# speedcell4/torchrua

Hardware: AMD Instinct MI355X
Metric: pack->reduce throughput, 65536 seqs/GPU h=512 bf16 (M elements/s) + % HBM roofline (higher is better)
Workload: dtype bf16; 1 GPU; pack->reduce_sum: 65536 seqs/GPU, len~U(8,512), hidden=512, bf16 (north-star shape; N=17046960 rows on rank 0); ranks_reported_by_process_group=1, cpus_of_rank0=256, torch_threads_rank0=16, numa_node_of_rank0_gpu=0

## Files before the change

### include/rua.h

```cpp
#ifndef RUA_H_
#define RUA_H_

#include <stdint.h>

#ifdef __cplusplus
extern "C" {
#endif

#define RUA_ABI_VERSION 6

#define RUA_EINVAL   (-1)
#define RUA_EALIGN   (-2)
#define RUA_ERANGE   (-3)

enum rua_kind { RUA_CAT = 0, RUA_LEFT = 1, RUA_PACK = 2, RUA_RIGHT = 3, RUA_LIST = 4 };

typedef struct rua_layout {
  int32_t kind;
  int32_t tile_t_log2;
  int64_t n_rows;
  int64_t B;
  int64_t T_phys;
  int64_t T_log;
  const int64_t* lens;
// ... 50 lines not shown
int rua_move_rows(const rua_layout* dst, const rua_layout* src, int32_t tmap, int64_t tmap_arg,
                  void* dst_data, const void* src_data, int64_t row_bytes,
                  const void* fill16, int64_t pad_row, int32_t flags, void* stream);

int rua_setitem_backward(const rua_layout* list, const rua_layout* src, const void* grad, void* grad_value,
                         void* grad_raw, int64_t row_bytes, int32_t flags, void* stream);

enum rua_dtype {
  RUA_F32 = 0, RUA_BF16 = 1, RUA_F16 = 2, RUA_F64 = 3,
  RUA_I64 = 4, RUA_I32 = 5, RUA_I16 = 6, RUA_I8 = 7, RUA_U8 = 8
};
#define RUA_TIES_FINAL 2
#define RUA_BWD_FILL_PADDING 0x100
#define RUA_BWD_TIES_POSITIVE 0x200
enum rua_op {
  RUA_SUM = 0, RUA_MEAN = 1, RUA_MAX = 2, RUA_MIN = 3, RUA_PROD = 4, RUA_LOGSUMEXP = 5
};

#define RUA_EXTREME_WORDS    1027
#define RUA_OP_SCRATCH_CLEAN 0x100
#define RUA_OP_NO_EMPTY      0x200
#define RUA_OP_SHORT_SEQS    0x400
int64_t rua_reduce_ws_bytes(int64_t n_rows, int64_t H, int32_t dtype, int64_t split_rows);
int rua_reduce_team_waves(int64_t n_rows, int64_t B, int64_t row_bytes);
int rua_segment_reduce(const rua_layout* lay, const int64_t* perm, const void* data, void* out,
                       int64_t H, int32_t dtype, int32_t op, int32_t include_self,
                       uint64_t empty_bits, void* extreme, int64_t split_rows, void* ws, void* ties_out,
                       void* stream);

int rua_pack_reduce(const rua_layout* src, const rua_layout* pack, const void* data, void* pack_data, void* out,
                    int64_t H, int32_t dtype, int32_t op, uint64_t empty_bits, void* extreme, int64_t split_rows,
                    void* ws, void* stream);

int rua_pack_sums(const rua_layout* src, const rua_layout* pack, const void* data, void* pack_data, float* sums,
                  int64_t H, int32_t dtype, int64_t split_rows, void* ws, void* stream);

int rua_pack_sums_backward(const rua_layout* src, const rua_layout* pack, const void* grad_pack, const float* grad_sums,
                           void* grad_src, int64_t H, int32_t dtype, void* stream);

int rua_sums_cast(const void* in, void* out, int64_t n, int32_t dtype, int32_t to_f32, void* stream);

int rua_segment_reduce_backward(const rua_layout* lay, const int64_t* perm, const void* data, const void* out,
                                const void* grad_out, void* grad_in, int64_t H, int32_t dtype, int32_t op,
                                int32_t include_self, int64_t split_rows, void* ws, void* ties,
                                const void* self_in, void* stream);

int rua_scatter_self_grad(const int64_t* counts, int64_t S, int64_t H, const void* self_in, const void* out,
                          const void* grad_out, const void* aux, void* grad_self, int32_t dtype, int32_t op,
                          int32_t include_self, void* stream);

int64_t rua_softmax_ws_bytes(const rua_layout* lay, int64_t H, int32_t dtype);
int rua_segment_softmax(const rua_layout* lay, const void* data, void* out, int64_t H, int32_t dtype, int32_t log,
                        void* ws, void* stream);
int rua_segment_softmax_backward(const rua_layout* lay, const void* y, const void* grad_out, void* grad_in, int64_t H,
                                 int32_t dtype, int32_t log, void* ws, void* stream);

#define RUA_POOL_OUT_ACC 0x100
int64_t rua_softmax_pool_ws_bytes(const rua_layout* lay, int64_t H, int64_t D, int32_t dtype);
int rua_segment_softmax_pool(const rua_layout* lay, const void* values, const void* scores, void* out, void* lse,
                             int64_t H, int64_t D, int32_t dtype, void* ws, void* stream);
int rua_segment_softmax_pool_backward(const rua_layout* lay, const void* grad_out, const void* values,
                                      const void* scores, const void* out, const void* lse, void* grad_values,
                                      void* grad_scores, int64_t H, int64_t D, int32_t dtype, void* ws, void* stream);

#define RUA_NORM_MEAN_ACC 0x100
int64_t rua_norm_ws_bytes(const rua_layout* lay, int64_t H, int32_t dtype);
// ... 156 lines not shown
```

### torchrua_amd/_lib.py

```python
import ctypes
import os
import threading
from ctypes import POINTER, Structure, c_char_p, c_double, c_int, c_int32, c_int64, c_uint64, c_void_p

import torch

_HERE = os.path.dirname(os.path.abspath(__file__))
LIB_PATH = os.environ.get('RUA_LIB_PATH') or os.path.join(_HERE, 'librua_hip.so')

ABI_VERSION = 6
CAT, LEFT, PACK, RIGHT, LIST = 0, 1, 2, 3, 4
T_SHIFT, T_ROLL, T_REV_S, T_REV_D, T_ZERO = 0, 1, 2, 3, 4
TIES_FINAL = 2
BWD_FILL_PADDING = 0x100
BWD_TIES_POSITIVE = 0x200
MOVE_SCATTER = 1
MOVE_NT_ON, MOVE_NT_OFF = 2, 4
MOVE_XCD_SPAN_ON, MOVE_XCD_SPAN_OFF = 256, 512
MOVE_NO_NARROW = 2048
OP_SCRATCH_CLEAN, OP_NO_EMPTY = 0x100, 0x200
EXTREME_WORDS = 1027
POOL_OUT_ACC = 0x100
NORM_MEAN_ACC = 0x100
OP_SHORT_SEQS = 0x400
CONV_MAX_TAPS = 8
JOIN_MAX_PARTS = 8
RUNS_BITS = 0x100
WINDOW_MAX_K = 64
CRF_MAX_TAGS = 64
CRF_LOG, CRF_MAX = 0, 1
WINDOW_TAKE = 6
F32, BF16, F16, F64 = 0, 1, 2, 3
SUM, MEAN, MAX, MIN, PROD, LOGSUMEXP = 0, 1, 2, 3, 4, 5

I64, I32, I16, I8, U8 = 4, 5, 6, 7, 8

DTYPES = {torch.float32: F32, torch.bfloat16: BF16, torch.float16: F16, torch.float64: F64}
INT_DTYPES = {torch.int64: I64, torch.int32: I32, torch.int16: I16, torch.int8: I8, torch.uint8: U8}
SCAN_DTYPES = {**DTYPES, torch.int64: I64}


class RuaLayout(Structure):
    _fields_ = [
        ('kind', c_int32), ('tile_t_log2', c_int32),
        ('n_rows', c_int64), ('B', c_int64), ('T_phys', c_int64), ('T_log', c_int64),
        ('lens', c_void_p), ('len_add', c_int64), ('off', c_void_p),
        ('boff', c_void_p), ('T', c_int64), ('sorted', c_void_p), ('unsorted', c_void_p),
        ('bptr', c_void_p), ('tptr', c_void_p),
        ('bsz', c_void_p), ('tile_start', c_void_p), ('n_tchunks', c_int64), ('n_tiles', c_int64),
    ]


# ... 200 lines not shown
```

### torchrua_amd/_ops.py

```python
import ctypes
import threading
from typing import Callable, Optional, Sequence, Tuple

import torch
from torch import Tensor
from torch.autograd.function import once_differentiable

from torchrua_amd import _lib as L
from torchrua_amd import _meta as M

_kernel_hook: Optional[Callable[[str, bool], None]] = None


def set_kernel_hook(fn) -> None:
    global _kernel_hook
    _kernel_hook = fn


def _prod(shape) -> int:
    n = 1
    for d in shape:
        n *= d
    return n

# ... 267 lines not shown
        split, ws = split_workspace(lay, H, data.dtype, dev, team_ok=False)
        L.check(lib.rua_segment_reduce_backward(lay.ref(), None, L.ptr(data), L.ptr(out), L.ptr(grad), L.ptr(g), H,
                                                L.DTYPES[data.dtype], op,
                                                (L.TIES_FINAL if ties is not None else 0) | L.BWD_FILL_PADDING | L.BWD_TIES_POSITIVE,
                                                split, L.ptr(ws), L.ptr(ties), None, L.stream_ptr(dev)),
                'rua_segment_reduce_backward')
        ctx.lay, ctx.op, ctx.hidden = lay, op, tuple(out.shape[1:])
        return g

    @staticmethod
    def backward(ctx, gg: Tensor):
        if ctx.op not in (L.SUM, L.MEAN):
            raise RuntimeError('torchrua_amd: prod (and the fused max / min / logsumexp kernel outside create_graph) '
                               'differentiate once; second-order gradients exist for sum, mean, max, min and logsumexp '
                               '(and for every cast, select and gather)')
        return reduce(gg.contiguous(), ctx.lay, ctx.op, ctx.hidden, None), None, None, None, None, None


def reduce(data: Tensor, lay: M.Lay, op: int, hidden, lens: Optional[Tensor]) -> Tensor:
    if data.requires_grad and torch.is_grad_enabled():
        return _Reduce.apply(data.contiguous(), lay, op, tuple(hidden), lens)
    return launch_reduce(lay, _plain(data), op, hidden=tuple(hidden))


SUMS_DTYPES = (torch.float32, torch.bfloat16, torch.float16)
_SUMS_KEY = 'pack_sums'


def pack_sums_can(data: Tensor, hidden: Tuple[int, ...]) -> bool:
    return (data.dtype in SUMS_DTYPES and data.is_contiguous() and data.data_ptr() % 16 == 0 and data.numel() > 0
            and (_prod(hidden) * data.element_size()) % 16 == 0)


def launch_pack_sums(data: Tensor, src: M.Lay, dst: M.Lay, hidden: Tuple[int, ...]) -> Tuple[Tensor, Tensor]:
    dev = data.device
    H = _prod(hidden)
    pdata = torch.empty((dst.n_rows,) + tuple(hidden), dtype=data.dtype, device=dev)
    sums = torch.empty((src.B,) + tuple(hidden), dtype=torch.float32, device=dev)
    split, ws = split_workspace(src, H, data.dtype, dev, team_ok=False)
    _call('to_pack', 'rua_pack_sums', dev, src.ref(), dst.ref(), L.ptr(data), L.ptr(pdata), L.ptr(sums), H,
          L.DTYPES[data.dtype], split, L.ptr(ws))
    return pdata, sums


def launch_sums_cast(x: Tensor, dtype: torch.dtype, to_f32: bool, name: Optional[str] = None) -> Tensor:
    dev = L.require_device(x)
    x = x.contiguous()
    out = torch.empty(x.shape, dtype=torch.float32 if to_f32 else dtype, device=dev)
    args = (L.ptr(x), L.ptr(out), x.numel(), L.DTYPES[dtype], 1 if to_f32 else 0)
    if name is None:
        L.check(L.load().rua_sums_cast(*args, L.stream_ptr(dev)), 'rua_sums_cast')
    else:
        _call(name, 'rua_sums_cast', dev, *args)
    return out


class _SumsCast(torch.autograd.Function):

    @staticmethod
    def forward(ctx, sums: Tensor, dtype: torch.dtype):
        ctx.dtype = dtype
        return launch_sums_cast(sums, dtype, False, name='reduce')

    @staticmethod
    def backward(ctx, grad: Tensor):
        if torch.is_grad_enabled():
            return grad.to(torch.float32), None
        return launch_sums_cast(grad, ctx.dtype, True), None


class _PackSums(torch.autograd.Function):

    @staticmethod
    def forward(ctx, data: Tensor, src: M.Lay, dst: M.Lay, hidden: Tuple[int, ...]):
# ... 1735 lines not shown
```

### torchrua_amd/csrc/rua_pack_sums_plan.h

```cpp
#pragma once
#include <stdint.h>
#include "rua.h"
#include "rua_wave.h"

namespace rua {

inline int pack_sums_check(const rua_layout* src, const rua_layout* pack, int64_t H, int32_t dtype) {
  if (!src || !pack || H < 0 || src->B < 0) return RUA_EINVAL;
  if (dtype != RUA_F32 && dtype != RUA_BF16 && dtype != RUA_F16) return RUA_EINVAL;
  if (src->kind != RUA_CAT && src->kind != RUA_LEFT && src->kind != RUA_RIGHT) return RUA_EINVAL;
  if (src->kind == RUA_CAT && src->lens && !src->off) return RUA_EINVAL;
  if (pack->kind != RUA_PACK || pack->B != src->B || (pack->T > 0 && !pack->boff)) return RUA_EINVAL;
  return 0;
}

struct PackSumsBackwardPlan {
  int err, epl, lp_log2;
  int64_t n_chunks;
  unsigned grid;
};
inline PackSumsBackwardPlan plan_pack_sums_backward(int64_t B, int64_t H, int esize, uintptr_t ptrs) {
  PackSumsBackwardPlan P = {};
  P.epl = 16 / esize;
  if (H % P.epl != 0 || ptrs % 16 != 0) { P.err = RUA_EALIGN; return P; }
  const int64_t lpr = H / P.epl;
  P.lp_log2 = lanes_log2(lpr);
  P.n_chunks = (lpr + RUA_WAVE - 1) / RUA_WAVE;
  if (B > 0x7fffffffLL / (P.n_chunks > 0 ? P.n_chunks : 1)) { P.err = RUA_ERANGE; return P; }
  P.grid = (unsigned)(B * P.n_chunks);
  return P;
}

}
```

### torchrua_amd/csrc/rua_reduce.hip

```cpp
#include <hip/hip_runtime.h>
#include <stdarg.h>
#include <stdio.h>
#include <string.h>
#include <atomic>
#include <deque>
#include <mutex>
#include <string>
#include "rua_reduce_impl.h"
#include "rua_pack_sums_plan.h"

namespace rua {
std::atomic<int> g_trace_on{0};
static std::mutex g_trace_mu;
static std::deque<std::string> g_trace_log;
constexpr size_t TRACE_CAP = 512;
static inline bool tracing() { return g_trace_on.load(std::memory_order_relaxed) != 0; }
void trace_add(const char* rec) {
  std::lock_guard<std::mutex> lk(g_trace_mu);
  if (g_trace_log.size() >= TRACE_CAP) g_trace_log.pop_front();
  g_trace_log.emplace_back(rec);
}
__attribute__((format(printf, 1, 2))) static std::string fmt(const char* f, ...) {
  char buf[320];
  va_list ap;
  va_start(ap, f);
  vsnprintf(buf, sizeof buf, f, ap);
  va_end(ap);
  return buf;
}
static const char* op_name(int op, bool ties) {
  switch (op) {
    case RUA_SUM: return "sum";
    case RUA_MEAN: return "mean";
    case RUA_MAX: return ties ? "max_t" : "max";
    case RUA_MIN: return ties ? "min_t" : "min";
    case RUA_PROD: return "prod";
    case RUA_LOGSUMEXP: return "logsumexp";
  }
  return "?";
}
template <typename Emit>
static void trace_reduce(const ReducePlan& P, const char* tname, Emit&& emit) {
  static const char* const kern[] = {"seg_reduce_ranks_kernel", "seg_reduce_team_kernel", "seg_reduce_kernel"};
  auto rec = [&](const char* k, bool nt, int wpb) {
    emit(fmt("%s T=%s EPL=%d OP=%s NT=%d COPY=%d CPW=%d WPB=%d team=%d glog=%d check=%d split=%d no_empty=%d", k, tname,
             P.epl, op_name(P.op, P.ties), nt ? 1 : 0, P.copy ? 1 : 0, P.cpw, wpb, P.team, P.glog, P.check,
             P.split ? 1 : 0, P.no_empty).c_str());
  };
  rec(kern[P.form], P.nt, P.wpb);
  if (P.split) {
    rec("seg_reduce_tail_kernel", P.nt, 1);
    rec("seg_reduce_combine_kernel", false, COMBINE_WAVES_MAX / P.cpw);
  }
}
template <typename Emit>
static void trace_backward(const BackwardPlan& P, const char* tname, Emit&& emit) {
  static const char* const kern[] = {"seg_backward_rows_kernel", "seg_backward_ranks_kernel", "seg_backward_walk_kernel",
                                     "seg_backward_kernel"};
  for (int k = 0; k < P.n_phases; ++k)
    for (const char* name : {kern[P.form], "seg_backward_tail_kernel"}) {
      emit(fmt("%s T=%s EPL=%d OP=%s NT=%d TV=%d chunks=%d span=%d split=%d phased=%d ties_final=%d pad_memset=%d", name,
               tname, P.epl, op_name(P.op, false), P.nt ? 1 : 0, P.tv[k], P.n_chunks > 1 ? 1 : 0, P.span ? 1 : 0,
               P.do_split ? 1 : 0, P.phased ? 1 : 0, P.ties_final ? 1 : 0, P.pad_memset ? 1 : 0).c_str());
      if (!P.do_split) break;
    }
}

static const ReduceEntry* entry_for(int dtype) {
  switch (dtype) {
    case RUA_F32: return &reduce_entry_f32();
    case RUA_BF16: return &reduce_entry_bf16();
    case RUA_F16: return &reduce_entry_f16();
    case RUA_F64: return &reduce_entry_f64();
  }
  return nullptr;
}

static int dispatch_reduce(int dtype, int op, hipStream_t s, const rua_layout& L, const int64_t* perm, const void* data,
                           void* out, int64_t H, int include_self, uint64_t empty_bits, void* extreme, int64_t split,
                           void* ws, const rua_layout* CD, void* copy, void* ties, int hints, std::string* dry,
                           void* acc_out = nullptr) {
  const ReduceEntry* E = entry_for(dtype);
  if (!E) return RUA_EINVAL;
  const ReducePlan P = plan_reduce(L, E->esize, H, op, include_self, perm != nullptr, ws != nullptr, ties != nullptr,
                                   copy != nullptr,
                                   (uintptr_t)data | (uintptr_t)out | (uintptr_t)copy | (uintptr_t)ties | (uintptr_t)acc_out,
                                   split, hints);
  if (P.err) return P.err;
  if (dry) trace_reduce(P, E->name, [&](const char* r) { dry->append(r).push_back('\n'); });
  else if (tracing()) trace_reduce(P, E->name, trace_add);
  return dry ? 0 : E->reduce(P, s, L, perm, data, out, H, include_self, empty_bits, extreme, ws, CD, copy, ties, acc_out);
}

constexpr int EXTREME_WORDS_ENTRY = RUA_EXTREME_WORDS;
__global__ void extreme_init_entry_kernel(unsigned long long* ext, int want_max_of_data) {
  (void)want_max_of_data;
  for (int i = threadIdx.x; i < EXTREME_WORDS_ENTRY; i += blockDim.x) ext[i] = 0ull;
}
int reduce_int(int dtype, int op, hipStream_t s, const rua_layout& L, const int64_t* perm, const void* data, void* out,
               int64_t H, int include_self, int64_t split, void* ws);
int64_t reduce_int_ws_bytes(int64_t n_rows, int64_t H, int64_t split);

static bool layout_ok(const rua_layout* lay, const int64_t* perm, int64_t H) {
  if (!lay || H < 0 || lay->B < 0) return false;
  if (lay->kind != RUA_CAT && lay->kind != RUA_PACK && lay->kind != RUA_LEFT && lay->kind != RUA_RIGHT) return false;
  if (lay->kind == RUA_CAT && lay->lens && !lay->off) return false;
  if (lay->kind == RUA_PACK && lay->T > 0 && !lay->boff) return false;
  return !perm || lay->kind == RUA_CAT;
}
static int segment_reduce_backward(const rua_layout* lay, const int64_t* perm, const void* data, const void* out,
                                   const void* grad_out, void* grad_in, int64_t H, int32_t dtype, int32_t op,
                                   int32_t include_self, int64_t split_rows, void* ws, void* ties, const void* self_in,
                                   void* stream, std::string* dry) {
  if (!layout_ok(lay, perm, H)) return RUA_EINVAL;
  if (self_in && !perm) return RUA_EINVAL;
  if (lay->B == 0 || H == 0 || lay->n_rows == 0) return 0;
  if (!data || !out || !grad_out || !grad_in) return RUA_EINVAL;
  const bool fill = (include_self & RUA_BWD_FILL_PADDING) != 0;
  const int tie_rule = (include_self & RUA_BWD_TIES_POSITIVE) ? BWD_TIES_POSITIVE : 0;
  include_self &= 0xff;
// ... 126 lines not shown
  if (include_self && op == RUA_PROD && !aux) return RUA_EINVAL;
  hipStream_t s = (hipStream_t)stream;
  const int inc = include_self ? 1 : 0;
  const ReduceEntry* E = entry_for(dtype);
  return E ? E->self_grad(s, counts, S, H, self_in, out, grad_out, aux, grad_self, op, inc) : RUA_EINVAL;
}

int64_t rua_reduce_ws_bytes(int64_t n_rows, int64_t H, int32_t dtype, int64_t split_rows) {
  if (split_rows <= 0 || n_rows <= 0 || H <= 0) return 0;
  if (dtype >= RUA_I64 && dtype <= RUA_U8) return reduce_int_ws_bytes(n_rows, H, split_rows);
  const int64_t acc = dtype == RUA_F64 ? 8 : 4;
  const int64_t max_extra = n_rows / split_rows;
  const int64_t chunks_scalar = (H + RUA_WAVE - 1) / RUA_WAVE;
  const int64_t max_u = max_extra * chunks_scalar;
  const int64_t cols = chunks_scalar * RUA_WAVE * (dtype == RUA_F64 ? 2 : 8);
  return 32 + max_u * 64 + 2 * max_extra * 2 * cols * acc + 256;
}

int rua_segment_reduce(const rua_layout* lay, const int64_t* perm, const void* data, void* out, int64_t H,
                       int32_t dtype, int32_t op, int32_t include_self, uint64_t empty_bits, void* extreme,
                       int64_t split_rows, void* ws, void* ties, void* stream) {
  return segment_reduce(lay, perm, data, out, H, dtype, op, include_self, empty_bits, extreme, split_rows, ws, ties, stream,
                        nullptr);
}

int rua_pack_reduce(const rua_layout* src, const rua_layout* pack, const void* data, void* pack_data, void* out,
                    int64_t H, int32_t dtype, int32_t op, uint64_t empty_bits, void* extreme, int64_t split_rows,
                    void* ws, void* stream) {
  return pack_reduce(src, pack, data, pack_data, out, H, dtype, op, empty_bits, extreme, split_rows, ws, stream, nullptr);
}

int rua_pack_sums(const rua_layout* src, const rua_layout* pack, const void* data, void* pack_data, float* sums,
                  int64_t H, int32_t dtype, int64_t split_rows, void* ws, void* stream) {
  const int rc = pack_sums_check(src, pack, H, dtype);
  if (rc) return rc;
  if (src->B == 0 || H == 0) return 0;
  if (!sums || !pack_data || !data) return RUA_EINVAL;
  return dispatch_reduce(dtype, RUA_SUM, (hipStream_t)stream, *src, nullptr, data, nullptr, H, 0, 0, nullptr, split_rows, ws,
                         pack, pack_data, nullptr, 0, nullptr, sums);
}

int rua_pack_sums_backward(const rua_layout* src, const rua_layout* pack, const void* grad_pack, const float* grad_sums,
                           void* grad_src, int64_t H, int32_t dtype, void* stream) {
  const int rc = pack_sums_check(src, pack, H, dtype);
  if (rc) return rc;
  if (src->B == 0 || H == 0 || src->n_rows == 0) return 0;
  if (!grad_pack || !grad_sums || !grad_src) return RUA_EINVAL;
  const ReduceEntry* E = entry_for(dtype);
  const PackSumsBackwardPlan P = plan_pack_sums_backward(src->B, H, E->esize,
                                                         (uintptr_t)grad_pack | (uintptr_t)grad_sums | (uintptr_t)grad_src);
  if (P.err) return P.err;
  const bool nt = reduce_nt(src->n_rows, H, E->esize);
  if (tracing())
    trace_add(fmt("pack_sums_backward_kernel T=%s EPL=%d NT=%d chunks=%lld", E->name, P.epl, nt ? 1 : 0,
                  (long long)P.n_chunks).c_str());
  return E->pack_sums_backward((hipStream_t)stream, *src, *pack, grad_pack, grad_sums, grad_src, H, P.lp_log2, P.n_chunks, nt);
}

int rua_sums_cast(const void* in, void* out, int64_t n, int32_t dtype, int32_t to_f32, void* stream) {
  if (n < 0 || (dtype != RUA_F32 && dtype != RUA_BF16 && dtype != RUA_F16)) return RUA_EINVAL;
  if (n == 0) return 0;
  if (!in || !out || in == out) return RUA_EINVAL;
  const ReduceEntry* E = entry_for(dtype);
  const uintptr_t narrow = (uintptr_t)(to_f32 ? in : out), wide = (uintptr_t)(to_f32 ? out : in);
  if (narrow % E->esize != 0 || wide % 4 != 0) return RUA_EALIGN;
  return E->sums_cast((hipStream_t)stream, in, out, n, to_f32 ? 1 : 0);
}

int rua_fill_empty(const rua_layout* lay, void* out, int64_t H, int32_t dtype, int32_t op, void* extreme,
                   void* stream) {
  if (!lay || H < 0 || !extreme) return RUA_EINVAL;
  const int reset = (op & RUA_OP_SCRATCH_CLEAN) ? 1 : 0;
// ... 19 lines not shown
```

### torchrua_amd/csrc/rua_reduce_impl.h

```cpp
#pragma once
#include <type_traits>
#include <hip/hip_bf16.h>
#include <hip/hip_fp16.h>
#include "rua_dev.h"
#include "rua_reduce_plan.h"

namespace rua {

constexpr int UNROLL_T = RUA_UNROLL_T;
constexpr int EXTREME_SLOTS = 1024;

template <typename T> struct elem;
template <> struct elem<float> {
  using acc = float;
  static __device__ __forceinline__ float up(float v) { return v; }
  static __device__ __forceinline__ float down(float v) { return v; }
};
template <> struct elem<double> {
  using acc = double;
  static __device__ __forceinline__ double up(double v) { return v; }
  static __device__ __forceinline__ double down(double v) { return v; }
};
template <> struct elem<__hip_bfloat16> {
  using acc = float;
// ... 95 lines not shown

constexpr int RUA_MAX_T = 6, RUA_MIN_T = 7;
constexpr bool op_is_max(int op) { return op == RUA_MAX || op == RUA_MAX_T; }
constexpr bool op_is_min(int op) { return op == RUA_MIN || op == RUA_MIN_T; }
constexpr bool op_counts(int op) { return op == RUA_MAX_T || op == RUA_MIN_T; }
constexpr bool op_uses_aux(int op) { return op == RUA_LOGSUMEXP || op_counts(op); }

template <typename A, bool IS_MAX>
__device__ __forceinline__ void tie_update(A& acc, A& cnt, A x, A c) {
  const bool xn = x != x, an = acc != acc;
  const bool better = xn ? !an : (!an && (IS_MAX ? x > acc : x < acc));
  const bool equal = xn ? an : (x == acc);
  cnt = better ? c : (equal ? cnt + c : cnt);
  acc = better ? x : acc;
}

template <typename A, int EPL>
struct Fold {
  A acc[EPL], aux[EPL];
  A opp;
};

template <typename A, int EPL, int OP>
__device__ __forceinline__ void fold_init(Fold<A, EPL>& f) {
#pragma unroll
  for (int e = 0; e < EPL; ++e) {
    f.acc[e] = (OP == RUA_PROD) ? (A)1 : (op_is_max(OP) || OP == RUA_LOGSUMEXP) ? -acc_inf<A>()
             : op_is_min(OP) ? acc_inf<A>() : (A)0;
    f.aux[e] = (A)0;
  }
  f.opp = op_is_min(OP) ? -acc_inf<A>() : acc_inf<A>();
}

template <typename T, int EPL, int OP, bool NT, bool COPY, int CPW = 1, bool RANKS = false>
__device__ __forceinline__ void fold_rows(const Unit<T, EPL>& U, int64_t t_lo, int64_t t_hi,
                                          const T* __restrict__ data, int64_t H,
                                          Fold<typename elem<T>::acc, EPL * CPW>& f, const rua_layout& CD,
                                          T* __restrict__ copy, int lane, int team_w = 0, int team_n = 1,
                                          bool track = true) {
  using A = typename elem<T>::acc;
  constexpr int UT = CPW == 1 ? UNROLL_T : UNROLL_T / 2;
  constexpr int CW = RUA_WAVE * EPL;
  struct alignas(sizeof(T) * EPL > 8 ? 8 : sizeof(T) * EPL) Pack { T v[EPL]; };
  typedef unsigned int RawV0 __attribute__((ext_vector_type(sizeof(T) * EPL >= 4 ? sizeof(T) * EPL / 4 : 1)));
  typedef RawV0 RawV __attribute__((aligned(sizeof(T) * EPL > 8 ? 8 : (sizeof(T) * EPL >= 4 ? sizeof(T) * EPL : 4))));
  const int rpw = U.rpw, rsub = U.rsub;
  const bool colok = U.colok;
  const int64_t col = U.col, base = U.base, tb = U.tb, L_rows = U.n_rows;
  const int64_t* __restrict__ tbl = U.tbl;

  int64_t tv = (tbl && t_lo + lane < t_hi) ? tbl[tb + t_lo + lane] : 0;
  int64_t cv = (COPY && t_lo + lane < t_hi) ? CD.boff[t_lo + lane] : 0;
  for (int64_t tblk = t_lo; tblk < t_hi; tblk += RUA_WAVE) {
    const int64_t nxt = tblk + RUA_WAVE + lane;
    const int64_t tv_next = (tbl && nxt < t_hi) ? tbl[tb + nxt] : 0;
    const int64_t cv_next = (COPY && nxt < t_hi) ? CD.boff[nxt] : 0;
    const int nblk = (t_hi - tblk) < RUA_WAVE ? (int)(t_hi - tblk) : RUA_WAVE;
    for (int k = 0; k < nblk; k += rpw * UT) {
      if (team_n > 1 && (int)(((tblk - t_lo) / (rpw * UT) + k / (rpw * UT)) % team_n) != team_w) continue;
      int64_t row[UT];
      int64_t crow[UT];
      Pack p[UT][CPW];
#pragma unroll
      for (int u = 0; u < UT; ++u) {
        const int tl = k + u * rpw + rsub;
        const int64_t tabv = __shfl(tv, tl & (RUA_WAVE - 1), RUA_WAVE);
        row[u] = -1;
        if (colok && tl < nblk && (!RANKS || tblk + tl < U.len)) row[u] = base + (tbl ? tabv : tblk + tl);
        if (row[u] >= L_rows) row[u] = -1;
        if (COPY) crow[u] = __shfl(cv, tl & (RUA_WAVE - 1), RUA_WAVE) + U.q;
      }
#pragma unroll
      for (int u = 0; u < UT; ++u)
#pragma unroll
        for (int c = 0; c < CPW; ++c)
          if (row[u] >= 0 && (CPW == 1 || col + c * CW < H)) {
            const T* src = data + row[u] * H + col + c * CW;
            if (NT && sizeof(Pack) >= 4) {
              RawV raw = __builtin_nontemporal_load(reinterpret_cast<const RawV*>(src));
              __builtin_memcpy(&p[u][c], &raw, sizeof(Pack));
            } else {
              p[u][c] = *reinterpret_cast<const Pack*>(src);
            }
          }
      if (COPY) {
#pragma unroll
        for (int u = 0; u < UT; ++u)
#pragma unroll
          for (int c = 0; c < CPW; ++c)
            if (row[u] >= 0 && crow[u] < CD.n_rows && (CPW == 1 || col + c * CW < H)) {
              T* dstp = copy + crow[u] * H + col + c * CW;
              if (NT && sizeof(Pack) >= 4) {
// ... 240 lines not shown
  }
  const unsigned long long want = (__any(nan) ? 1ull : 0ull) | (__any(empty_unit) ? 2ull : 0ull);
  if (lane != 0) return;
  if (track && opp == opp && opp != (op_is_min(OP) ? -acc_inf<A>() : acc_inf<A>())) {
    const unsigned long long bits = (unsigned long long)ordered_bits(opp);
    atomicMax(&extreme[extreme_slot()], op_is_min(OP) ? bits : ~bits);
  }
  if (want == 0ull) return;
  const unsigned long long have = __atomic_load_n(&extreme[EXTREME_SLOTS], __ATOMIC_RELAXED);
  if ((have & want) != want) atomicOr(&extreme[EXTREME_SLOTS], want);
}

struct SplitWs {
  unsigned long long* ctr;
  int64_t* long_list;
  int64_t* items;
  void* partials;
  int64_t max_u;
  int64_t split;
  void* ties;
  void* acc_out;
};

template <typename A, int EPL, int OP>
__device__ __forceinline__ void store_partial(void* partials, int64_t slot, int lane, const Fold<A, EPL>& f) {
  A* p = reinterpret_cast<A*>(partials) + (slot * 2 * RUA_WAVE + lane) * EPL;
#pragma unroll
  for (int e = 0; e < EPL; ++e) {
    p[e] = f.acc[e];
    if (op_uses_aux(OP)) p[RUA_WAVE * EPL + e] = f.aux[e];
  }
}

template <typename T, int EPL, int OP, bool NT, bool COPY, bool SPLIT, int CPW, int WPB = 1>
__global__ __launch_bounds__(RUA_WAVE * WPB) void seg_reduce_kernel(rua_layout L, const int64_t* __restrict__ perm,
                                                              const T* __restrict__ data, T* __restrict__ out,
                                                              int64_t H, int lp_log2, int64_t n_chunks,
                                                              int include_self, T empty_val,
                                                              unsigned long long* __restrict__ extreme,
                                                              rua_layout CD, T* __restrict__ copy, SplitWs W,
                                                              int no_empty) {
  using A = typename elem<T>::acc;
  const int lane = threadIdx.x & (RUA_WAVE - 1);
  const int64_t wid = (int64_t)blockIdx.x * WPB + (threadIdx.x >> 6);
  const int64_t q = wid / n_chunks;
  if (q >= L.B) return;
  constexpr int NE = EPL * CPW;
  const Unit<T, EPL> U = make_unit<T, EPL, COPY, CPW>(L, CD, perm, q, wid - q * n_chunks, H, lp_log2, lane);
  Fold<A, NE> f;
  fold_init<A, NE, OP>(f);
  const bool track = track_initial<OP>(L, extreme, no_empty);

  if (SPLIT && U.len > W.split) {
    const int64_t nparts = (U.len + W.split - 1) / W.split;
    int64_t pbase = 0, ibase = 0;
    if (lane == 0) {
      const unsigned long long old = atomicAdd(&W.ctr[0], (1ull << 32) | (unsigned long long)(nparts - 1));
      ibase = (int64_t)(old & 0xffffffffull);
      const int64_t li = (int64_t)(old >> 32);
      pbase = ibase + li;
      int64_t* e = W.long_list + li * 4;
      e[0] = q; e[1] = U.chunk; e[2] = nparts; e[3] = pbase;
    }
    pbase = __shfl(pbase, 0, RUA_WAVE);
    ibase = __shfl(ibase, 0, RUA_WAVE);
    for (int64_t p = 1 + lane; p < nparts; p += RUA_WAVE) {
      int64_t* e = W.items + (ibase + p - 1) * 4;
      e[0] = q; e[1] = U.chunk; e[2] = p; e[3] = pbase + p;
    }
    fold_rows<T, EPL, OP, NT, COPY, CPW>(U, 0, W.split, data, H, f, CD, copy, lane, 0, 1, track);
    fold_wave<A, NE, OP>(f, lp_log2);
    store_partial<A, NE, OP>(W.partials, pbase, lane, f);
  } else {
    fold_rows<T, EPL, OP, NT, COPY, CPW>(U, 0, U.len, data, H, f, CD, copy, lane, 0, 1, track);
    fold_wave<A, NE, OP>(f, lp_log2);
    fold_store<T, EPL, OP, CPW>(U, f, out, H, include_self, empty_val, (A*)W.ties, COPY ? (A*)W.acc_out : nullptr);
  }
  fold_flags<A, NE, OP>(f, extreme, lane, U.len <= 0, track);
}

constexpr int TEAM_MAX = 4;
template <typename T, int EPL, int OP, bool NT>
__global__ __launch_bounds__(RUA_WAVE * TEAM_MAX) void seg_reduce_team_kernel(
    rua_layout L, const int64_t* __restrict__ perm, const T* __restrict__ data, T* __restrict__ out, int64_t H,
    int lp_log2, int64_t n_chunks, int include_self, T empty_val, unsigned long long* __restrict__ extreme,
    typename elem<T>::acc* __restrict__ ties, int no_empty) {
  using A = typename elem<T>::acc;
  __shared__ A s_acc[TEAM_MAX][RUA_WAVE * EPL];
  __shared__ A s_aux[TEAM_MAX][RUA_WAVE * EPL];
  const int lane = threadIdx.x & (RUA_WAVE - 1), wave = threadIdx.x >> 6, team = blockDim.x >> 6;
  const int64_t wid = blockIdx.x;
  const int64_t q = wid / n_chunks;
  if (q >= L.B) return;
  const Unit<T, EPL> U = make_unit<T, EPL, false, 1>(L, L, perm, q, wid - q * n_chunks, H, lp_log2, lane);
  Fold<A, EPL> f;
  fold_init<A, EPL, OP>(f);
  const bool track = track_initial<OP>(L, extreme, no_empty);
  fold_rows<T, EPL, OP, NT, false, 1>(U, 0, U.len, data, H, f, L, nullptr, lane, wave, team, track);
  fold_wave<A, EPL, OP>(f, lp_log2);
  fold_flags<A, EPL, OP>(f, extreme, lane, wave == 0 && U.len <= 0, track);
  if (wave > 0) {
#pragma unroll
    for (int k = 0; k < EPL; ++k) { s_acc[wave][lane * EPL + k] = f.acc[k]; s_aux[wave][lane * EPL + k] = f.aux[k]; }
  }
  __syncthreads();
  if (wave == 0) {
    for (int w = 1; w < team; ++w) {
      A a2[EPL], x2[EPL];
#pragma unroll
      for (int k = 0; k < EPL; ++k) { a2[k] = s_acc[w][lane * EPL + k]; x2[k] = s_aux[w][lane * EPL + k]; }
      fold_merge<A, EPL, OP>(f, a2, x2);
// ... 882 lines not shown
      return;
    }
    with_epl<T>(P.epl, [&](auto epl_c) {
      constexpr int EPL = decltype(epl_c)::value;
      with_bool(P.nt, [&](auto nt_c) {
        constexpr bool NT = decltype(nt_c)::value;
        if constexpr (!NT || EPL == FULL) {
          if (P.form == REDUCE_RANKS) {
            if (!P.split) {
              hipLaunchKernelGGL((seg_reduce_ranks_kernel<T, EPL, OP, NT>), g, b, 0, s, L, (const T*)data, (T*)out, H,
                                 lp_log2, include_self, ev, ext, (A*)ties, P.glog, W, no_empty, P.check);
            } else if constexpr (EPL == FULL) {
              hipLaunchKernelGGL((seg_reduce_ranks_kernel<T, EPL, OP, NT, true>), g, b, 0, s, L, (const T*)data, (T*)out,
                                 H, lp_log2, include_self, ev, ext, (A*)ties, P.glog, W, no_empty, P.check);
              split_rest(epl_c, nt_c, std::false_type{}, int_c<1>{});
            }
            return;
          }
          with_bool(P.copy, [&](auto copy_c) {
            constexpr bool COPY = decltype(copy_c)::value;
            with_bool(P.cpw == 4, [&](auto wide_c) {
              constexpr int CPW = decltype(wide_c)::value ? 4 : 1;
              if constexpr ((!COPY || (EPL == FULL && !op_counts(OP))) && (CPW == 1 || EPL == FULL || EPL == HALF)) {
                if (P.split) {
                  hipLaunchKernelGGL((seg_reduce_kernel<T, EPL, OP, NT, COPY, true, CPW>), g, b, 0, s, L, perm,
                                     (const T*)data, (T*)out, H, lp_log2, n_chunks, include_self, ev, ext, cd, (T*)copy, W,
                                     no_empty);
                  split_rest(epl_c, nt_c, copy_c, int_c<CPW>{});
                } else if (P.wpb == 2) {
                  if constexpr (!COPY && CPW == 1)
                    hipLaunchKernelGGL((seg_reduce_kernel<T, EPL, OP, NT, COPY, false, CPW, 2>), dim3((P.grid + 1) / 2),
                                       dim3(RUA_WAVE * 2), 0, s, L, perm, (const T*)data, (T*)out, H, lp_log2, n_chunks,
                                       include_self, ev, ext, cd, (T*)copy, W, no_empty);
                } else {
                  hipLaunchKernelGGL((seg_reduce_kernel<T, EPL, OP, NT, COPY, false, CPW>), g, b, 0, s, L, perm,
                                     (const T*)data, (T*)out, H, lp_log2, n_chunks, include_self, ev, ext, cd, (T*)copy, W,
                                     no_empty);
                }
              }
            });
          });
        }
      });
    });
  });
  return rc ? rc : (int)hipGetLastError();
}

template <typename T>
static int launch_backward(const BackwardPlan& P, hipStream_t s, const rua_layout& L, const int64_t* perm,
                           const void* data, const void* out, const void* gout, void* gin, int64_t H, int extra_count,
                           void* ws, void* ties, const void* self_in) {
  using A = typename elem<T>::acc;
  constexpr int FULL = 16 / sizeof(T);
  if (P.pad_memset) {
    const hipError_t e = hipMemsetAsync(gin, 0, (size_t)L.n_rows * (size_t)H * sizeof(T), s);
    if (e != hipSuccess) return (int)e;
  }
  const T *xp = (const T*)data, *op_ = (const T*)out, *gp = (const T*)gout, *sp = (const T*)self_in;
  T* ip = (T*)gin;
  A* tp = (A*)ties;
  const int lp_log2 = P.lp_log2, tie_rule = extra_count & BWD_TIES_POSITIVE;
  const int64_t n_chunks = P.n_chunks;
  SplitWs W = {};
  if (P.do_split) W = carve_ws<A>(ws, P.max_u, P.split_rows);
  const dim3 g(P.grid), b(RUA_WAVE);
// ... 98 lines not shown
```

### torchrua_amd/csrc/rua_reduce_plan.h

```cpp
#pragma once
#include <stdint.h>
#include "rua.h"
#include "rua_wave.h"

namespace rua {

#ifndef RUA_UNROLL_T
#define RUA_UNROLL_T 8
#endif
constexpr int REDUCE_UNROLL_T = RUA_UNROLL_T;
constexpr int64_t REDUCE_TEAM_MAX_UNITS = 16384;
constexpr int COMBINE_WAVES_MAX = 16;
constexpr int REDUCE_HINT_NO_EMPTY = 1, REDUCE_HINT_SHORT_SEQS = 2;
constexpr int64_t RANKS_MIN_WAVES = 4096;
constexpr int64_t RANKS_MIN_WAVES_SHORT = 512;
constexpr int COMBINE_SOLO = 32;
constexpr int64_t COMBINE_GRID = 512;
constexpr int BROWS_MAX = 256;
constexpr int64_t SPLIT_GRID_CAP = 16384;
constexpr int BWD_SELF_COUNTS = 1, BWD_TIES_POSITIVE = 2;

inline int reduce_team_waves(int64_t n_rows, int64_t B, int lp_log2, int64_t units, int unroll_t = REDUCE_UNROLL_T) {
  if (units <= 0 || units > REDUCE_TEAM_MAX_UNITS) return 1;
  const int64_t rows_per_group = (int64_t)(RUA_WAVE >> lp_log2) * unroll_t;
  const int64_t groups = n_rows / (B > 0 ? B : 1) / rows_per_group;
  return groups >= 4 * 4 ? 4 : groups >= 4 * 2 ? 2 : 1;
}

inline bool reduce_nt(int64_t n_rows, int64_t H, int esize) {
  return (double)n_rows * (double)H * (double)esize >= (double)(512ll << 20);
}
inline int64_t split_max_extra(int64_t n_rows, int64_t split) { return split > 0 ? n_rows / split : 0; }
inline unsigned split_grid(int64_t max_u) { return (unsigned)(max_u < SPLIT_GRID_CAP ? max_u : SPLIT_GRID_CAP); }

enum { REDUCE_RANKS, REDUCE_TEAM, REDUCE_SEQ };
struct ReducePlan {
  int err;
  int form, esize, op, epl, lp_log2, cpw, wpb, team, glog, check, no_empty;
  bool ties, nt, copy, split;
  int64_t n_chunks, split_rows, max_u;
  unsigned grid;
};

enum { BWD_ROWS, BWD_RANKS, BWD_WALK, BWD_SEQ };
struct BackwardPlan {
  int err;
  int form, esize, op, epl, lp_log2, n_phases, tv[2], tile_rows;
  bool nt, span, do_split, phased, ties_final, pad_memset;
  int64_t n_chunks, per_xcd, split_rows, max_u;
  unsigned grid;
};

inline ReducePlan plan_reduce(const rua_layout& L, int esize, int64_t H, int op, int include_self, bool perm, bool ws,
                              bool ties, bool copy, uintptr_t ptrs, int64_t split, int hints) {
  ReducePlan P = {};
  P.form = REDUCE_SEQ; P.esize = esize; P.op = op; P.team = 1; P.copy = copy; P.ties = ties && !copy;
  P.no_empty = (hints & REDUCE_HINT_NO_EMPTY) ? 1 : 0; P.split_rows = split;
  const bool short_seqs = (hints & REDUCE_HINT_SHORT_SEQS) != 0;
  if (op < RUA_SUM || op > RUA_LOGSUMEXP) { P.err = RUA_EINVAL; return P; }
  const int FULL = 16 / esize;
  const int HALF = FULL >= 4 ? FULL / 2 : 1;
  const bool aligned_ok = (H % FULL == 0) && (ptrs % 16 == 0);
  const bool tail_ok = !aligned_ok && FULL > 1 && H > FULL && (H + FULL - 1) / FULL <= RUA_WAVE &&
                       (H * (int64_t)esize) % 8 == 0 && (ptrs % 8 == 0) && include_self != 1 && !copy;
  const bool vec_ok = aligned_ok || tail_ok;
  const bool half_ok = !vec_ok && HALF > 1 && (H % HALF == 0) && (ptrs % 8 == 0);
  P.epl = vec_ok ? FULL : half_ok ? HALF : 1;
  const int64_t lpr = (H + P.epl - 1) / P.epl;
  const int lp_log2 = P.lp_log2 = lanes_log2(lpr);
  const bool wide = (vec_ok || (half_ok && L.kind == RUA_PACK)) && lpr > RUA_WAVE;
  P.cpw = wide ? 4 : 1;
  P.n_chunks = (lpr + RUA_WAVE * P.cpw - 1) / (RUA_WAVE * P.cpw);
  const int64_t blocks = L.B * P.n_chunks;
  if (blocks > 0x7fffffffLL) { P.err = RUA_ERANGE; return P; }
  P.nt = vec_ok && reduce_nt(L.n_rows, H, esize);
  P.grid = (unsigned)blocks;
  if (copy && !aligned_ok) { P.err = RUA_EALIGN; return P; }
  bool cat_ranks = L.kind == RUA_CAT && L.lens && L.len_add == 0 && lp_log2 < 6;
  int glog = 0;
  if (cat_ranks) {
    const int64_t side = RUA_WAVE >> lp_log2;
    const int64_t short_avg = 4 * side < 16 ? 16 : (4 * side > 64 ? 64 : 4 * side);
    if (L.n_rows > short_avg * L.B) {
      if (lp_log2 <= 1) glog = 4 - lp_log2;
      else cat_ranks = false;
    }
    if (cat_ranks && glog == 0 && lp_log2 <= 1 && (L.B >> (6 - lp_log2)) < RANKS_MIN_WAVES_SHORT) glog = 4 - lp_log2;
  }
  const bool short_form = (cat_ranks && glog == 0) || (L.kind == RUA_PACK && L.T > 0 && L.T <= 128);
  const int64_t ranks_min_waves = short_form ? RANKS_MIN_WAVES_SHORT : RANKS_MIN_WAVES;
  const int ranks_check = (cat_ranks && !short_seqs) ? 1 : 0;
  const bool ranks_split = split > 0 && ws && cat_ranks && (glog > 0 || ranks_check) && vec_ok && split_max_extra(L.n_rows, split) > 0;
  if (((L.kind == RUA_PACK && L.sorted) || cat_ranks) && !copy && !perm && lp_log2 < 6 && (!(split > 0 && ws) || ranks_split) &&
      (L.B >> (6 - lp_log2 - glog)) >= ranks_min_waves) {
    const int64_t rpw = RUA_WAVE >> (lp_log2 + glog);
    const int64_t nblk = (L.B + rpw - 1) / rpw;
    if (nblk > 0x7fffffffLL) { P.err = RUA_ERANGE; return P; }
    P.form = REDUCE_RANKS; P.wpb = 1; P.glog = glog; P.check = ranks_check; P.split = ranks_split;
    P.grid = (unsigned)nblk;
    P.max_u = ranks_split ? split_max_extra(L.n_rows, split) : 0;
    if (P.max_u > 0x7fffffffLL) P.err = RUA_ERANGE;
    return P;
  }
  if (vec_ok && !wide && !copy && !(split > 0 && ws)) {
    const int team = reduce_team_waves(L.n_rows, L.B, lp_log2, blocks);
    if (team > 1) {
      P.form = REDUCE_TEAM; P.wpb = P.team = team;
      return P;
    }
  }
  P.max_u = split_max_extra(L.n_rows, split) * P.n_chunks;
  P.split = split > 0 && ws && P.max_u > 0;
  if (P.split && P.max_u > 0x7fffffffLL) { P.err = RUA_ERANGE; return P; }
  P.wpb = (copy || P.cpw != 1 || P.split) ? 1 : ((L.kind != RUA_PACK && H * (int64_t)esize >= 512) ? 2 : 1);
  return P;
}

inline BackwardPlan plan_backward(const rua_layout& L, int esize, int64_t H, int op, int extra_count, bool perm, bool ws,
                                  bool ties, bool ties_final, bool self_in, bool fill_padding, uintptr_t ptrs,
                                  int64_t split) {
  BackwardPlan P = {};
  P.form = BWD_SEQ; P.esize = esize; P.op = op; P.n_phases = 1; P.ties_final = ties_final; P.split_rows = split;
  if (op < RUA_SUM || op > RUA_LOGSUMEXP) { P.err = RUA_EINVAL; return P; }
  const int FULL = 16 / esize;
  const int HALF = FULL >= 4 ? FULL / 2 : 1;
  const bool vec_ok = (H % FULL == 0) && (ptrs % 16 == 0);
  const bool half_ok = !vec_ok && HALF > 1 && (H % HALF == 0) && (ptrs % 8 == 0);
  P.epl = vec_ok ? FULL : half_ok ? HALF : 1;
  const int64_t lpr = (H + P.epl - 1) / P.epl;
  const int lp_log2 = P.lp_log2 = lanes_log2(lpr);
  P.n_chunks = (lpr + RUA_WAVE - 1) / RUA_WAVE;
  const int64_t blocks = L.B * P.n_chunks;
  if (blocks > 0x7fffffffLL) { P.err = RUA_ERANGE; return P; }
  P.grid = (unsigned)blocks;
  const bool extreme_op = op == RUA_MAX || op == RUA_MIN;
  const bool rows_op = op == RUA_SUM || op == RUA_MEAN || op == RUA_LOGSUMEXP || (extreme_op && ties && ties_final);
  const bool plain = !perm && !self_in && !(extra_count & BWD_SELF_COUNTS);
  if (vec_ok && plain && rows_op && L.kind != RUA_PACK && H * (int64_t)esize >= 64) {
    const int64_t row_bytes = H * (int64_t)esize;
    P.tile_rows = BROWS_MAX;
    for (int64_t tb = BROWS_MAX * row_bytes; P.tile_rows > 4 && tb > (16 << 10); tb >>= 1) P.tile_rows >>= 1;
    const int64_t ntiles = (L.n_rows + P.tile_rows - 1) / P.tile_rows;
    P.span = ntiles >= 2048;
    P.per_xcd = P.span ? (ntiles + 7) / 8 : 0;
    const int64_t grid = P.span ? P.per_xcd * 8 : ntiles;
    if (grid > 0x7fffffffLL) { P.err = RUA_ERANGE; return P; }
    P.form = BWD_ROWS; P.grid = (unsigned)grid; P.nt = reduce_nt(L.n_rows, H, esize);
// ... 28 lines not shown
```

Baseline: 1.399 million M elements/s.

## Add lockstep group form for pack-sums copy reduce with barrier-synchronized waves

Adds a GRP template parameter to seg_reduce_kernel so groups of 4/8/16 adjacent sequences run as waves in one workgroup. The waves iterate in lockstep up to the group's maximum length, with an s_barrier per step. The aim is to keep the scattered packed-layout writes of neighbouring sequences close together in time for better DRAM/cache locality. By default the planner picks group width 4 when rows are at least 512 bytes and there are at least 16384 units. A Python setter can override the width. The cost is barrier overhead, plus idle waves that loop to the group's longest sequence.

Result: slower. 1.335 million M elements/s (-4.6%).

```diff
diff --git a/include/rua.h b/include/rua.h
--- a/include/rua.h
+++ b/include/rua.h
@@ -106,6 +106,8 @@
                     int64_t H, int32_t dtype, int32_t op, uint64_t empty_bits, void* extreme, int64_t split_rows,
                     void* ws, void* stream);
 
+#define RUA_PACK_SUMS_GROUP(g) ((g) == 1 ? 0x100 : (g) == 4 ? 0x200 : (g) == 8 ? 0x300 : (g) == 16 ? 0x400 : 0x700)
+#define RUA_PACK_SUMS_GROUP_MASK 0x700
 int rua_pack_sums(const rua_layout* src, const rua_layout* pack, const void* data, void* pack_data, float* sums,
                   int64_t H, int32_t dtype, int64_t split_rows, void* ws, void* stream);
 
diff --git a/torchrua_amd/_lib.py b/torchrua_amd/_lib.py
--- a/torchrua_amd/_lib.py
+++ b/torchrua_amd/_lib.py
@@ -18,6 +18,7 @@
 MOVE_NT_ON, MOVE_NT_OFF = 2, 4
 MOVE_XCD_SPAN_ON, MOVE_XCD_SPAN_OFF = 256, 512
 MOVE_NO_NARROW = 2048
+PACK_SUMS_GROUP = {1: 0x100, 4: 0x200, 8: 0x300, 16: 0x400}
 OP_SCRATCH_CLEAN, OP_NO_EMPTY = 0x100, 0x200
 EXTREME_WORDS = 1027
 POOL_OUT_ACC = 0x100
diff --git a/torchrua_amd/_ops.py b/torchrua_amd/_ops.py
--- a/torchrua_amd/_ops.py
+++ b/torchrua_amd/_ops.py
@@ -323,14 +323,25 @@
             and (_prod(hidden) * data.element_size()) % 16 == 0)
 
 
+_pack_sums_group: Optional[int] = None
+
+
+def set_pack_sums_group(group: Optional[int]) -> None:
+    global _pack_sums_group
+    if group is not None and group not in L.PACK_SUMS_GROUP:
+        raise ValueError(f'pack_sums group width: None or one of {sorted(L.PACK_SUMS_GROUP)}; got {group!r}')
+    _pack_sums_group = group
+
+
 def launch_pack_sums(data: Tensor, src: M.Lay, dst: M.Lay, hidden: Tuple[int, ...]) -> Tuple[Tensor, Tensor]:
     dev = data.device
     H = _prod(hidden)
     pdata = torch.empty((dst.n_rows,) + tuple(hidden), dtype=data.dtype, device=dev)
     sums = torch.empty((src.B,) + tuple(hidden), dtype=torch.float32, device=dev)
     split, ws = split_workspace(src, H, data.dtype, dev, team_ok=False)
+    code = L.DTYPES[data.dtype] | (L.PACK_SUMS_GROUP[_pack_sums_group] if _pack_sums_group is not None else 0)
     _call('to_pack', 'rua_pack_sums', dev, src.ref(), dst.ref(), L.ptr(data), L.ptr(pdata), L.ptr(sums), H,
-          L.DTYPES[data.dtype], split, L.ptr(ws))
+          code, split, L.ptr(ws))
     return pdata, sums
 
 
diff --git a/torchrua_amd/csrc/rua_pack_sums_plan.h b/torchrua_amd/csrc/rua_pack_sums_plan.h
--- a/torchrua_amd/csrc/rua_pack_sums_plan.h
+++ b/torchrua_amd/csrc/rua_pack_sums_plan.h
@@ -12,6 +12,17 @@
   if (src->kind == RUA_CAT && src->lens && !src->off) return RUA_EINVAL;
   if (pack->kind != RUA_PACK || pack->B != src->B || (pack->T > 0 && !pack->boff)) return RUA_EINVAL;
   return 0;
+}
+
+inline int pack_sums_group(int32_t dtype) {
+  switch (dtype & RUA_PACK_SUMS_GROUP_MASK) {
+    case 0: return 0;
+    case RUA_PACK_SUMS_GROUP(1): return 1;
+    case RUA_PACK_SUMS_GROUP(4): return 4;
+    case RUA_PACK_SUMS_GROUP(8): return 8;
+    case RUA_PACK_SUMS_GROUP(16): return 16;
+  }
+  return -1;
 }
 
 struct PackSumsBackwardPlan {
diff --git a/torchrua_amd/csrc/rua_reduce.hip b/torchrua_amd/csrc/rua_reduce.hip
--- a/torchrua_amd/csrc/rua_reduce.hip
+++ b/torchrua_amd/csrc/rua_reduce.hip
@@ -42,15 +42,15 @@
 template <typename Emit>
 static void trace_reduce(const ReducePlan& P, const char* tname, Emit&& emit) {
   static const char* const kern[] = {"seg_reduce_ranks_kernel", "seg_reduce_team_kernel", "seg_reduce_kernel"};
-  auto rec = [&](const char* k, bool nt, int wpb) {
-    emit(fmt("%s T=%s EPL=%d OP=%s NT=%d COPY=%d CPW=%d WPB=%d team=%d glog=%d check=%d split=%d no_empty=%d", k, tname,
-             P.epl, op_name(P.op, P.ties), nt ? 1 : 0, P.copy ? 1 : 0, P.cpw, wpb, P.team, P.glog, P.check,
-             P.split ? 1 : 0, P.no_empty).c_str());
+  auto rec = [&](const char* k, bool nt, int wpb, int grp) {
+    emit(fmt("%s T=%s EPL=%d OP=%s NT=%d COPY=%d CPW=%d WPB=%d team=%d glog=%d check=%d split=%d no_empty=%d GRP=%d", k,
+             tname, P.epl, op_name(P.op, P.ties), nt ? 1 : 0, P.copy ? 1 : 0, P.cpw, wpb, P.team, P.glog, P.check,
+             P.split ? 1 : 0, P.no_empty, grp).c_str());
   };
-  rec(kern[P.form], P.nt, P.wpb);
+  rec(kern[P.form], P.nt, P.wpb, P.grp);
   if (P.split) {
-    rec("seg_reduce_tail_kernel", P.nt, 1);
-    rec("seg_reduce_combine_kernel", false, COMBINE_WAVES_MAX / P.cpw);
+    rec("seg_reduce_tail_kernel", P.nt, 1, 1);
+    rec("seg_reduce_combine_kernel", false, COMBINE_WAVES_MAX / P.cpw, 1);
   }
 }
 template <typename Emit>
@@ -79,13 +79,13 @@
 static int dispatch_reduce(int dtype, int op, hipStream_t s, const rua_layout& L, const int64_t* perm, const void* data,
                            void* out, int64_t H, int include_self, uint64_t empty_bits, void* extreme, int64_t split,
                            void* ws, const rua_layout* CD, void* copy, void* ties, int hints, std::string* dry,
-                           void* acc_out = nullptr) {
+                           void* acc_out = nullptr, int group = 0) {
   const ReduceEntry* E = entry_for(dtype);
   if (!E) return RUA_EINVAL;
   const ReducePlan P = plan_reduce(L, E->esize, H, op, include_self, perm != nullptr, ws != nullptr, ties != nullptr,
                                    copy != nullptr,
                                    (uintptr_t)data | (uintptr_t)out | (uintptr_t)copy | (uintptr_t)ties | (uintptr_t)acc_out,
-                                   split, hints);
+                                   split, hints, group);
   if (P.err) return P.err;
   if (dry) trace_reduce(P, E->name, [&](const char* r) { dry->append(r).push_back('\n'); });
   else if (tracing()) trace_reduce(P, E->name, trace_add);
@@ -278,12 +278,14 @@
 
 int rua_pack_sums(const rua_layout* src, const rua_layout* pack, const void* data, void* pack_data, float* sums,
                   int64_t H, int32_t dtype, int64_t split_rows, void* ws, void* stream) {
-  const int rc = pack_sums_check(src, pack, H, dtype);
+  const int group = pack_sums_group(dtype);
+  dtype &= ~RUA_PACK_SUMS_GROUP_MASK;
+  const int rc = group < 0 ? RUA_EINVAL : pack_sums_check(src, pack, H, dtype);
   if (rc) return rc;
   if (src->B == 0 || H == 0) return 0;
   if (!sums || !pack_data || !data) return RUA_EINVAL;
   return dispatch_reduce(dtype, RUA_SUM, (hipStream_t)stream, *src, nullptr, data, nullptr, H, 0, 0, nullptr, split_rows, ws,
-                         pack, pack_data, nullptr, 0, nullptr, sums);
+                         pack, pack_data, nullptr, 0, nullptr, sums, group);
 }
 
 int rua_pack_sums_backward(const rua_layout* src, const rua_layout* pack, const void* grad_pack, const float* grad_sums,
diff --git a/torchrua_amd/csrc/rua_reduce_impl.h b/torchrua_amd/csrc/rua_reduce_impl.h
--- a/torchrua_amd/csrc/rua_reduce_impl.h
+++ b/torchrua_amd/csrc/rua_reduce_impl.h
@@ -151,12 +151,12 @@
   f.opp = op_is_min(OP) ? -acc_inf<A>() : acc_inf<A>();
 }
 
-template <typename T, int EPL, int OP, bool NT, bool COPY, int CPW = 1, bool RANKS = false>
+template <typename T, int EPL, int OP, bool NT, bool COPY, int CPW = 1, bool RANKS = false, int GRP = 1>
 __device__ __forceinline__ void fold_rows(const Unit<T, EPL>& U, int64_t t_lo, int64_t t_hi,
                                           const T* __restrict__ data, int64_t H,
                                           Fold<typename elem<T>::acc, EPL * CPW>& f, const rua_layout& CD,
                                           T* __restrict__ copy, int lane, int team_w = 0, int team_n = 1,
-                                          bool track = true) {
+                                          bool track = true, int64_t t_sync = 0) {
   using A = typename elem<T>::acc;
   constexpr int UT = CPW == 1 ? UNROLL_T : UNROLL_T / 2;
   constexpr int CW = RUA_WAVE * EPL;
@@ -170,13 +170,16 @@
 
   int64_t tv = (tbl && t_lo + lane < t_hi) ? tbl[tb + t_lo + lane] : 0;
   int64_t cv = (COPY && t_lo + lane < t_hi) ? CD.boff[t_lo + lane] : 0;
-  for (int64_t tblk = t_lo; tblk < t_hi; tblk += RUA_WAVE) {
+  const int64_t t_end = GRP > 1 ? t_sync : t_hi;
+  for (int64_t tblk = t_lo; tblk < t_end; tblk += RUA_WAVE) {
     const int64_t nxt = tblk + RUA_WAVE + lane;
     const int64_t tv_next = (tbl && nxt < t_hi) ? tbl[tb + nxt] : 0;
     const int64_t cv_next = (COPY && nxt < t_hi) ? CD.boff[nxt] : 0;
-    const int nblk = (t_hi - tblk) < RUA_WAVE ? (int)(t_hi - tblk) : RUA_WAVE;
-    for (int k = 0; k < nblk; k += rpw * UT) {
-      if (team_n > 1 && (int)(((tblk - t_lo) / (rpw * UT) + k / (rpw * UT)) % team_n) != team_w) continue;
+    const int nblk = (t_hi - tblk) < RUA_WAVE ? (GRP > 1 && t_hi < tblk ? 0 : (int)(t_hi - tblk)) : RUA_WAVE;
+    const int ntrip = GRP > 1 ? ((t_end - tblk) < RUA_WAVE ? (int)(t_end - tblk) : RUA_WAVE) : nblk;
+    for (int k = 0; k < ntrip; k += rpw * UT) {
+      if (GRP > 1) __builtin_amdgcn_s_barrier();
+      if (GRP == 1 && team_n > 1 && (int)(((tblk - t_lo) / (rpw * UT) + k / (rpw * UT)) % team_n) != team_w) continue;
       int64_t row[UT];
       int64_t crow[UT];
       Pack p[UT][CPW];
@@ -483,8 +486,8 @@
   }
 }
 
-template <typename T, int EPL, int OP, bool NT, bool COPY, bool SPLIT, int CPW, int WPB = 1>
-__global__ __launch_bounds__(RUA_WAVE * WPB) void seg_reduce_kernel(rua_layout L, const int64_t* __restrict__ perm,
+template <typename T, int EPL, int OP, bool NT, bool COPY, bool SPLIT, int CPW, int WPB = 1, int GRP = 1>
+__global__ __launch_bounds__(RUA_WAVE * WPB * GRP) void seg_reduce_kernel(rua_layout L, const int64_t* __restrict__ perm,
                                                               const T* __restrict__ data, T* __restrict__ out,
                                                               int64_t H, int lp_log2, int64_t n_chunks,
                                                               int include_self, T empty_val,
@@ -493,11 +496,33 @@
                                                               int no_empty) {
   using A = typename elem<T>::acc;
   const int lane = threadIdx.x & (RUA_WAVE - 1);
-  const int64_t wid = (int64_t)blockIdx.x * WPB + (threadIdx.x >> 6);
-  const int64_t q = wid / n_chunks;
-  if (q >= L.B) return;
+  const int64_t wid = (int64_t)blockIdx.x * (WPB * GRP) + (threadIdx.x >> 6);
+  int64_t q = wid / n_chunks;
   constexpr int NE = EPL * CPW;
-  const Unit<T, EPL> U = make_unit<T, EPL, COPY, CPW>(L, CD, perm, q, wid - q * n_chunks, H, lp_log2, lane);
+  bool live = true;
+  int64_t t_sync = 0;
+  if constexpr (GRP > 1) {
+    static_assert(COPY && !SPLIT && CPW == 1 && WPB == 1 && GRP <= RUA_WAVE, "the lockstep group form: plan_reduce");
+    const int64_t q0 = (int64_t)blockIdx.x * GRP;
+    int64_t glen = 0;
+    if (lane < GRP && q0 + lane < L.B) {
+      int64_t b = CD.sorted ? CD.sorted[q0 + lane] : q0 + lane;
+      if (b < 0 || b >= L.B) b = q0 + lane;
+      glen = seq_len(L, b);
+    }
+#pragma unroll
+    for (int d = GRP / 2; d > 0; d >>= 1) {
+      const int64_t o = __shfl_xor(glen, d, RUA_WAVE);
+      glen = o > glen ? o : glen;
+    }
+    t_sync = __shfl(glen, 0, RUA_WAVE);
+    live = q < L.B;
+    if (!live) q = L.B - 1;
+  } else {
+    if (q >= L.B) return;
+  }
+  Unit<T, EPL> U = make_unit<T, EPL, COPY, CPW>(L, CD, perm, q, GRP > 1 ? 0 : wid - q * n_chunks, H, lp_log2, lane);
+  if (GRP > 1 && !live) { U.len = 0; U.colok = false; }
   Fold<A, NE> f;
   fold_init<A, NE, OP>(f);
   const bool track = track_initial<OP>(L, extreme, no_empty);
@@ -523,11 +548,11 @@
     fold_wave<A, NE, OP>(f, lp_log2);
     store_partial<A, NE, OP>(W.partials, pbase, lane, f);
   } else {
-    fold_rows<T, EPL, OP, NT, COPY, CPW>(U, 0, U.len, data, H, f, CD, copy, lane, 0, 1, track);
+    fold_rows<T, EPL, OP, NT, COPY, CPW, false, GRP>(U, 0, U.len, data, H, f, CD, copy, lane, 0, 1, track, t_sync);
     fold_wave<A, NE, OP>(f, lp_log2);
     fold_store<T, EPL, OP, CPW>(U, f, out, H, include_self, empty_val, (A*)W.ties, COPY ? (A*)W.acc_out : nullptr);
   }
-  fold_flags<A, NE, OP>(f, extreme, lane, U.len <= 0, track);
+  fold_flags<A, NE, OP>(f, extreme, lane, live && U.len <= 0, track);
 }
 
 constexpr int TEAM_MAX = 4;
@@ -1476,6 +1501,16 @@
                     hipLaunchKernelGGL((seg_reduce_kernel<T, EPL, OP, NT, COPY, false, CPW, 2>), dim3((P.grid + 1) / 2),
                                        dim3(RUA_WAVE * 2), 0, s, L, perm, (const T*)data, (T*)out, H, lp_log2, n_chunks,
                                        include_self, ev, ext, cd, (T*)copy, W, no_empty);
+                } else if (P.grp > 1) {
+                  if constexpr (COPY && CPW == 1 && EPL == FULL && OP == RUA_SUM && sizeof(T) <= 4) {
+                    auto group = [&](auto grp_c) {
+                      constexpr int GRP = decltype(grp_c)::value;
+                      hipLaunchKernelGGL((seg_reduce_kernel<T, EPL, OP, NT, COPY, false, CPW, 1, GRP>),
+                                         dim3(reduce_workgroups(P)), dim3(RUA_WAVE * GRP), 0, s, L, perm, (const T*)data,
+                                         (T*)out, H, lp_log2, n_chunks, include_self, ev, ext, cd, (T*)copy, W, no_empty);
+                    };
+                    if (P.grp == 4) group(int_c<4>{}); else if (P.grp == 8) group(int_c<8>{}); else group(int_c<16>{});
+                  }
                 } else {
                   hipLaunchKernelGGL((seg_reduce_kernel<T, EPL, OP, NT, COPY, false, CPW>), g, b, 0, s, L, perm,
                                      (const T*)data, (T*)out, H, lp_log2, n_chunks, include_self, ev, ext, cd, (T*)copy, W,
diff --git a/torchrua_amd/csrc/rua_reduce_plan.h b/torchrua_amd/csrc/rua_reduce_plan.h
--- a/torchrua_amd/csrc/rua_reduce_plan.h
+++ b/torchrua_amd/csrc/rua_reduce_plan.h
@@ -18,6 +18,9 @@
 constexpr int64_t COMBINE_GRID = 512;
 constexpr int BROWS_MAX = 256;
 constexpr int64_t SPLIT_GRID_CAP = 16384;
+constexpr int64_t COPY_GROUP_MIN_UNITS = 16384;
+constexpr int COPY_GROUP_WIDTH = 4;
+inline bool copy_group_width_ok(int g) { return g == 4 || g == 8 || g == 16; }
 constexpr int BWD_SELF_COUNTS = 1, BWD_TIES_POSITIVE = 2;
 
 inline int reduce_team_waves(int64_t n_rows, int64_t B, int lp_log2, int64_t units, int unroll_t = REDUCE_UNROLL_T) {
@@ -37,10 +40,15 @@
 struct ReducePlan {
   int err;
   int form, esize, op, epl, lp_log2, cpw, wpb, team, glog, check, no_empty;
+  int grp;
   bool ties, nt, copy, split;
   int64_t n_chunks, split_rows, max_u;
   unsigned grid;
 };
+inline unsigned reduce_workgroups(const ReducePlan& P) {
+  const unsigned w = P.grp > 1 ? (unsigned)P.grp : P.wpb == 2 ? 2u : 1u;
+  return P.grid / w + (P.grid % w ? 1u : 0u);
+}
 
 enum { BWD_ROWS, BWD_RANKS, BWD_WALK, BWD_SEQ };
 struct BackwardPlan {
@@ -52,9 +60,10 @@
 };
 
 inline ReducePlan plan_reduce(const rua_layout& L, int esize, int64_t H, int op, int include_self, bool perm, bool ws,
-                              bool ties, bool copy, uintptr_t ptrs, int64_t split, int hints) {
+                              bool ties, bool copy, uintptr_t ptrs, int64_t split, int hints, int group = 0) {
   ReducePlan P = {};
-  P.form = REDUCE_SEQ; P.esize = esize; P.op = op; P.team = 1; P.copy = copy; P.ties = ties && !copy;
+  P.form = REDUCE_SEQ; P.esize = esize; P.op = op; P.team = 1; P.copy = copy; P.ties = ties && !copy; P.grp = 1;
+  if (group != 0 && group != 1 && !copy_group_width_ok(group)) { P.err = RUA_EINVAL; return P; }
   P.no_empty = (hints & REDUCE_HINT_NO_EMPTY) ? 1 : 0; P.split_rows = split;
   const bool short_seqs = (hints & REDUCE_HINT_SHORT_SEQS) != 0;
   if (op < RUA_SUM || op > RUA_LOGSUMEXP) { P.err = RUA_EINVAL; return P; }
@@ -113,6 +122,9 @@
   P.split = split > 0 && ws && P.max_u > 0;
   if (P.split && P.max_u > 0x7fffffffLL) { P.err = RUA_ERANGE; return P; }
   P.wpb = (copy || P.cpw != 1 || P.split) ? 1 : ((L.kind != RUA_PACK && H * (int64_t)esize >= 512) ? 2 : 1);
+  const bool grp_can = copy && op == RUA_SUM && esize <= 4 && P.epl == FULL && P.cpw == 1 && P.n_chunks == 1 && !P.split;
+  const bool grp_rule = H * (int64_t)esize >= 512 && blocks >= COPY_GROUP_MIN_UNITS;
+  if (grp_can) P.grp = group > 1 ? group : (group == 0 && grp_rule) ? COPY_GROUP_WIDTH : 1;
   return P;
 }
 
```
